# HansiZeng/RIPOR

Measured on AMD Instinct MI355X. Metric: queries/sec, t5-base beam=10 len=32 over 8.8M-doc trie (constrained beam search), higher is better.
Workload: dtype f32 via f16x2-split MFMA (fp32 accumulate)

## Files before the change

### ripor_amd/csrc/gemm_h2.hip

```cpp
#include <algorithm>
#include <cstdio>
#include <type_traits>
#include <hip/hip_fp16.h>

#include <cstdlib>

#include "common.h"
#include "gemm_route.h"

#include <algorithm>
#include <vector>

namespace rpr {

typedef _Float16 f16x8 __attribute__((ext_vector_type(8)));
typedef __bf16 bf16x8 __attribute__((ext_vector_type(8)));
typedef float f32x16 __attribute__((ext_vector_type(16)));
typedef float f32x4 __attribute__((ext_vector_type(4)));
typedef float f32x2 __attribute__((ext_vector_type(2)));
typedef _Float16 f16x2 __attribute__((ext_vector_type(2)));

template <bool M16, int TM, int TN> struct H2Acc { typedef f32x16 type[TM][TN]; };
template <int TM, int TN> struct H2Acc<true, TM, TN> { typedef f32x4 type[2 * TM][2 * TN]; };

// ... 68 lines not shown
      __half* dst = smem + (size_t)buf * ROWS * HBK + 16 * (wave + NW * j) * HBK;
      __builtin_amdgcn_global_load_lds((const __attribute__((address_space(1))) void*)(src[j] + k0),
                                       (__attribute__((address_space(3))) void*)dst, 16, 0, 0);
    }
  };

  f32x16 acc[TM][TN];
#pragma unroll
  for (int i = 0; i < TM; ++i)
#pragma unroll
    for (int j = 0; j < TN; ++j)
#pragma unroll
      for (int r = 0; r < 16; ++r) acc[i][j][r] = 0.f;

  const int frow = lane & 31, sw = (lane >> 2) & 3, hf = lane >> 5;
  const int a_row = wm * (BM / WM) + frow, w_row = 2 * BM + wn * (BN / WN) + frow;

  auto compute = [&](int buf) {
    const __half* base = smem + (size_t)buf * ROWS * HBK;
#pragma unroll
    for (int c = 0; c < HBK / 16; ++c) {
      const int so = ((2 * c + hf) ^ sw) * 8;
      if (BF16) {
        bf16x8 a0[TM], a1[TM], b0[TN], b1[TN];
#pragma unroll
        for (int i = 0; i < TM; ++i) {
          a0[i] = *reinterpret_cast<const bf16x8*>(base + (a_row + i * 32) * HBK + so);
          a1[i] = *reinterpret_cast<const bf16x8*>(base + (BM + a_row + i * 32) * HBK + so);
        }
#pragma unroll
        for (int j = 0; j < TN; ++j) {
          b0[j] = *reinterpret_cast<const bf16x8*>(base + (w_row + j * 32) * HBK + so);
          b1[j] = *reinterpret_cast<const bf16x8*>(base + (BN + w_row + j * 32) * HBK + so);
        }
#pragma unroll
        for (int i = 0; i < TM; ++i)
#pragma unroll
          for (int j = 0; j < TN; ++j) acc[i][j] = __builtin_amdgcn_mfma_f32_32x32x16_bf16(a0[i], b0[j], acc[i][j], 0, 0, 0);
#pragma unroll
        for (int i = 0; i < TM; ++i)
#pragma unroll
          for (int j = 0; j < TN; ++j) acc[i][j] = __builtin_amdgcn_mfma_f32_32x32x16_bf16(a1[i], b1[j], acc[i][j], 0, 0, 0);
        continue;
      }
      f16x8 ah[TM], al[TM], bh[TN], bl[TN];
#pragma unroll
      for (int i = 0; i < TM; ++i) {
        ah[i] = *reinterpret_cast<const f16x8*>(base + (a_row + i * 32) * HBK + so);
        al[i] = *reinterpret_cast<const f16x8*>(base + (BM + a_row + i * 32) * HBK + so);
      }
#pragma unroll
      for (int j = 0; j < TN; ++j) {
        bh[j] = *reinterpret_cast<const f16x8*>(base + (w_row + j * 32) * HBK + so);
        bl[j] = *reinterpret_cast<const f16x8*>(base + (BN + w_row + j * 32) * HBK + so);
      }
#pragma unroll
      for (int i = 0; i < TM; ++i)
#pragma unroll
        for (int j = 0; j < TN; ++j) acc[i][j] = __builtin_amdgcn_mfma_f32_32x32x16_f16(al[i], bh[j], acc[i][j], 0, 0, 0);
#pragma unroll
      for (int i = 0; i < TM; ++i)
#pragma unroll
        for (int j = 0; j < TN; ++j) acc[i][j] = __builtin_amdgcn_mfma_f32_32x32x16_f16(ah[i], bl[j], acc[i][j], 0, 0, 0);
#pragma unroll
      for (int i = 0; i < TM; ++i)
#pragma unroll
        for (int j = 0; j < TN; ++j) acc[i][j] = __builtin_amdgcn_mfma_f32_32x32x16_f16(ah[i], bh[j], acc[i][j], 0, 0, 0);
    }
  };

  if (STAGES == 2) {
    stage(0, 0);
    __syncthreads();
    for (int kt = 0; kt + 1 < nkt; ++kt) {
      stage((kt + 1) & 1, (kt + 1) * KSTEP);
      compute(kt & 1);
      __syncthreads();
    }
    compute((nkt - 1) & 1);
  } else {
    constexpr int AHEAD = STAGES - 1;
    static_assert(PER_WAVE * (AHEAD - 1) <= 63, "vmcnt is a 6-bit counter");
    constexpr int KEEP = PER_WAVE * (AHEAD - 1);
    constexpr int WAIT_KEEP = (KEEP & 15) | ((KEEP >> 4) << 14) | 0x0f70;
    constexpr int WAIT_NONE = 0x0f70;
#pragma unroll
    for (int t = 0; t < AHEAD; ++t)
      if (t < nkt) stage(t, t * KSTEP);
    for (int kt = 0; kt < nkt; ++kt) {
      if (kt + AHEAD - 1 < nkt) __builtin_amdgcn_s_waitcnt(WAIT_KEEP); else __builtin_amdgcn_s_waitcnt(WAIT_NONE);
      __builtin_amdgcn_s_barrier();
      __builtin_amdgcn_sched_barrier(0);
      if (kt + AHEAD < nkt) stage((kt + AHEAD) % STAGES, (kt + AHEAD) * KSTEP);
      compute(kt % STAGES);
      __builtin_amdgcn_sched_barrier(0);
    }
  }

  if (BF16) {
    constexpr int SH = BM / WM, SW = BN / WN;
    static_assert((size_t)BM * BN * sizeof(float) <= sizeof(smem), "the strips of all waves fit the operand buffers");
    __syncthreads();
    float* stg = reinterpret_cast<float*>(smem) + (size_t)wave * (SH * SW);
    const int ncol_ = lane & 31, rsub_ = 4 * (lane >> 5);
#pragma unroll
    for (int i = 0; i < TM; ++i)
#pragma unroll
      for (int j = 0; j < TN; ++j)
#pragma unroll
        for (int r = 0; r < 16; ++r) stg[(i * 32 + (r & 3) + 8 * (r >> 2) + rsub_) * SW + j * 32 + ncol_] = acc[i][j][r];
    __builtin_amdgcn_s_waitcnt(0xc07f);
    __builtin_amdgcn_wave_barrier();
    constexpr int LPR = SW / 4, RPI = 64 / LPR, NK = SH / RPI;
    const int rrow = lane / LPR, rc4 = (lane % LPR) * 4;
    const int mrow0 = bm + wm * SH, n0 = bn + wn * SW + rc4;
    const bool ncol_ok = FULL || n0 < g.N;
    float* outp = g.out[0] + (size_t)blockIdx.y * g.part_stride;
    const int ldo = g.ldo[0];
    const float relu_lo = g.relu ? 0.f : -INFINITY;
    float4 res[NK];
    if (g.resid) {
#pragma unroll
      for (int k = 0; k < NK; ++k) {
        const int m = min(mrow0 + k * RPI + rrow, g.M - 1), nc = ncol_ok ? n0 : 0;
        res[k] = *reinterpret_cast<const float4*>(g.resid + (size_t)m * g.ldr + nc);
      }
    }
#pragma unroll
    for (int k = 0; k < NK; ++k) {
      const int rl = k * RPI + rrow, m = mrow0 + rl;
      float4 v = *reinterpret_cast<const float4*>(stg + rl * SW + rc4);
      v.x = fmaxf(v.x * acc_scale, relu_lo); v.y = fmaxf(v.y * acc_scale, relu_lo);
      v.z = fmaxf(v.z * acc_scale, relu_lo); v.w = fmaxf(v.w * acc_scale, relu_lo);
      if (g.resid) { v.x = res[k].x + v.x; v.y = res[k].y + v.y; v.z = res[k].z + v.z; v.w = res[k].w + v.w; }
      if (ncol_ok && (FULL || m < g.M)) *reinterpret_cast<float4*>(outp + (size_t)m * ldo + n0) = v;
    }
    return;
  }
  int lane_e = lane;
  asm volatile("" : "+v"(lane_e));
  h2_epilogue_256<FULL, TM, TN, WM, WN, BM, BN>(g, acc, smem, wave, lane_e, bm, bn, wm, wn, g.row_ssq ? rs_tile : nullptr, acc_scale);
}

template <bool FULL, int TM, int TN, int WM, int WN, int strip, int BM = 256, int BN = 256, bool BOUT = false, bool M16 = false>
__device__ __forceinline__ void h2_epilogue_strip(const GemmH2Args& g, typename H2Acc<M16, TM, TN>::type& acc, float* stg, int lane, int bm, int bn,
                                                  int wm, int wn, const float* rs_tile, float acc_scale, int Mlim) {
  constexpr int SH = 64, SW = TN * 32;
  const int ncol = lane & 31, rsub = 4 * (lane >> 5);
  if constexpr (M16) {
    const int c16 = lane & 15, r16 = 4 * (lane >> 4);
#pragma unroll
    for (int ii = 0; ii < SH / 16; ++ii)
#pragma unroll
      for (int j = 0; j < 2 * TN; ++j)
#pragma unroll
        for (int r = 0; r < 4; ++r)
          stg[(ii * 16 + r16 + r) * SW + j * 16 + c16] = acc[strip * (SH / 16) + ii][j][r];
  } else
#pragma unroll
    for (int ii = 0; ii < SH / 32; ++ii)
#pragma unroll
      for (int j = 0; j < TN; ++j)
#pragma unroll
        for (int r = 0; r < 16; ++r)
          stg[(ii * 32 + (r & 3) + 8 * (r >> 2) + rsub) * SW + j * 32 + ncol] = acc[strip * (SH / 32) + ii][j][r];
    __builtin_amdgcn_s_waitcnt(0xc07f);
    __builtin_amdgcn_wave_barrier();
    const int mrow0 = bm + wm * (BM / WM) + strip * SH;
    auto planes_path = [&](auto res_tag) __attribute__((always_inline)) {
      constexpr bool RES = decltype(res_tag)::value;
      constexpr int LPR = SW / 8, RPI = 64 / LPR, NK = SH / RPI, KB = RES ? 2 : 4;
      const int rrow = lane / LPR, rc8 = (lane % LPR) * 8;
      const int n0 = bn + wn * (BN / WN) + rc8;
      const bool ncol_ok = FULL || (n0 < g.N);
      const float ps = g.plane_scale;
      float amax = 0.f;
      uint4 rh[RES ? NK : 1], rl_[RES ? NK : 1];
      if (RES) {
#pragma unroll
        for (int k = 0; k < NK; ++k) {
          const int m = min(mrow0 + k * RPI + rrow, Mlim - 1), nc = ncol_ok ? n0 : 0;
          rh[k] = *reinterpret_cast<const uint4*>(g.resid_h + (size_t)m * g.ldrh + nc);
          rl_[k] = *reinterpret_cast<const uint4*>(g.resid_h + g.r_ps + (size_t)m * g.ldrh + nc);
        }
      }
#pragma unroll
      for (int kb = 0; kb < NK; kb += KB) {
        float4 sa[KB], sb[KB];
        float scs[KB];
#pragma unroll
        for (int k = 0; k < KB; ++k) {
          const int rl = (kb + k) * RPI + rrow;
          sa[k] = *reinterpret_cast<const float4*>(stg + rl * SW + rc8);
          sb[k] = *reinterpret_cast<const float4*>(stg + rl * SW + rc8 + 4);
          scs[k] = rs_tile ? rs_tile[wm * (BM / WM) + strip * SH + rl] : 1.0f;
        }
        __builtin_amdgcn_sched_barrier(0);
#pragma unroll
        for (int k = 0; k < KB; ++k) {
          const int rl = (kb + k) * RPI + rrow, m = mrow0 + rl;
          const bool ok = ncol_ok && (FULL || m < Mlim);
          const float sc = rs_tile ? acc_scale * scs[k] : acc_scale;
          f32x2 v[4];
          *reinterpret_cast<float4*>(&v[0]) = sa[k];
          *reinterpret_cast<float4*>(&v[2]) = sb[k];
          f16x2 h[4], l[4];
          f32x2 ss2 = {0.f, 0.f};
          float am = 0.f;
#pragma unroll
          for (int e = 0; e < 4; ++e) {
            f32x2 x = v[e] * sc;
            if (g.relu) { x.x = fmaxf(x.x, 0.f); x.y = fmaxf(x.y, 0.f); }
            if (RES) {
              x += (__builtin_convertvector(reinterpret_cast<const f16x2*>(&rh[RES ? kb + k : 0])[e], f32x2) +
                    __builtin_convertvector(reinterpret_cast<const f16x2*>(&rl_[RES ? kb + k : 0])[e], f32x2)) * (1.0f / X_PLANE_SCALE);
            }
            ss2 += x * x;
            f32x2 xs = x * ps;
            am = fmaxf(am, fmaxf(fabsf(xs.x), fabsf(xs.y)));
            xs.x = __builtin_amdgcn_fmed3f(xs.x, -65504.f, 65504.f);
            xs.y = __builtin_amdgcn_fmed3f(xs.y, -65504.f, 65504.f);
            h[e] = __builtin_convertvector(xs, f16x2);
            l[e] = __builtin_convertvector(xs - __builtin_convertvector(h[e], f32x2), f16x2);
          }
          float ss = ss2.x + ss2.y;
          if (ok) {
            *reinterpret_cast<uint4*>(g.out_h + (size_t)m * g.ldoh + n0) = *reinterpret_cast<uint4*>(h);
            *reinterpret_cast<uint4*>(g.out_h + g.o_ps + (size_t)m * g.ldoh + n0) = *reinterpret_cast<uint4*>(l);
            amax = fmaxf(amax, am);
          }
          if (g.ssq_out) {
            if (!ok) ss = 0.f;
#pragma unroll
            for (int o = LPR / 2; o > 0; o >>= 1) ss += __shfl_xor(ss, o, 64);
            if ((lane % LPR) == 0 && (FULL || m < Mlim)) atomicAdd(g.ssq_out + m, ssq_to_fix(ss, g.sat));
          }
        }
      }
      if (amax > 65504.f && g.sat) *g.sat = 1u;
    };
    auto fp32_path = [&](auto res_tag, auto kv_tag) __attribute__((always_inline)) {
      constexpr bool RES = decltype(res_tag)::value, KVMAP = decltype(kv_tag)::value;
      const float relu_lo = g.relu ? 0.f : -INFINITY;
      constexpr int LPR = SW / 4, RPI = 64 / LPR, NK = SH / RPI, KB = RES ? 4 : 8;
      const int rrow = lane / LPR, rc4 = (lane % LPR) * 4;
      const int n0 = bn + wn * (BN / WN) + rc4;
      const bool ncol_ok = FULL || (n0 < g.N);
      const int oi = ncol_ok ? n0 / g.split_n : 0, on = n0 - oi * g.split_n;
      float* outp = (oi == 0 ? g.out[0] : oi == 1 ? g.out[1] : g.out[2]) + (size_t)blockIdx.y * g.part_stride;
      const int ldo = oi == 0 ? g.ldo[0] : oi == 1 ? g.ldo[1] : g.ldo[2];
      float4 res[RES ? NK : 1];
      if (RES) {
#pragma unroll
        for (int k = 0; k < NK; ++k) {
          const int m = min(mrow0 + k * RPI + rrow, Mlim - 1), nc = ncol_ok ? n0 : 0;
          res[k] = *reinterpret_cast<const float4*>(g.resid + (size_t)m * g.ldr + nc);
        }
      }
#pragma unroll
      for (int kb = 0; kb < NK; kb += KB) {
        float4 st[KB];
        float scs[KB];
#pragma unroll
        for (int k = 0; k < KB; ++k) {
          const int rl = (kb + k) * RPI + rrow;
          st[k] = *reinterpret_cast<const float4*>(stg + rl * SW + rc4);
          scs[k] = rs_tile ? rs_tile[wm * (BM / WM) + strip * SH + rl] : 1.0f;
        }
        __builtin_amdgcn_sched_barrier(0);
#pragma unroll
        for (int k = 0; k < KB; ++k) {
          const int rl = (kb + k) * RPI + rrow, m = mrow0 + rl;
          float4 v = st[k];
          const float sc = acc_scale * scs[k];
          v.x = fmaxf(v.x * sc, relu_lo); v.y = fmaxf(v.y * sc, relu_lo); v.z = fmaxf(v.z * sc, relu_lo); v.w = fmaxf(v.w * sc, relu_lo);
          if (RES) { const float4 r = res[RES ? kb + k : 0]; v.x = r.x + v.x; v.y = r.y + v.y; v.z = r.z + v.z; v.w = r.w + v.w; }
          if (ncol_ok && (FULL || m < Mlim)) {
            const size_t off = KVMAP ? out_off(g, oi, m, ldo, on) : (size_t)m * ldo + on;
            *reinterpret_cast<float4*>(outp + off) = v;
          }
        }
      }
    };
    auto bf16_path = [&](auto mask_tag) __attribute__((always_inline)) {
      constexpr bool MASK = decltype(mask_tag)::value;
      constexpr int LPR = SW / 8, RPI = 64 / LPR, NK = SH / RPI, KB = MASK ? 2 : 4;
      const int rrow = lane / LPR, rc8 = (lane % LPR) * 8;
      const int n0 = bn + wn * (BN / WN) + rc8;
      const float relu_lo = g.relu ? 0.f : -INFINITY;
      __bf16* ob = reinterpret_cast<__bf16*>(g.out_b);
      float* of = g.out[0];
      float4 ma[MASK ? NK : 1], mb[MASK ? NK : 1];
      if (MASK) {
#pragma unroll
        for (int k = 0; k < NK; ++k) {
          const float* mp = g.mask_src + (size_t)(mrow0 + k * RPI + rrow) * g.ldmask + n0;
          ma[k] = *reinterpret_cast<const float4*>(mp);
          mb[k] = *reinterpret_cast<const float4*>(mp + 4);
        }
      }
#pragma unroll
      for (int kb = 0; kb < NK; kb += KB) {
        float4 sa[KB], sb[KB];
#pragma unroll
        for (int k = 0; k < KB; ++k) {
          const int rl = (kb + k) * RPI + rrow;
          sa[k] = *reinterpret_cast<const float4*>(stg + rl * SW + rc8);
          sb[k] = *reinterpret_cast<const float4*>(stg + rl * SW + rc8 + 4);
        }
        __builtin_amdgcn_sched_barrier(0);
#pragma unroll
        for (int k = 0; k < KB; ++k) {
          const int rl = (kb + k) * RPI + rrow, m = mrow0 + rl;
          float v[8] = {sa[k].x, sa[k].y, sa[k].z, sa[k].w, sb[k].x, sb[k].y, sb[k].z, sb[k].w};
#pragma unroll
          for (int e = 0; e < 8; ++e) v[e] = fmaxf(v[e] * acc_scale, relu_lo);
          if (MASK) {
            const float mk[8] = {ma[MASK ? kb + k : 0].x, ma[MASK ? kb + k : 0].y, ma[MASK ? kb + k : 0].z, ma[MASK ? kb + k : 0].w,
                                 mb[MASK ? kb + k : 0].x, mb[MASK ? kb + k : 0].y, mb[MASK ? kb + k : 0].z, mb[MASK ? kb + k : 0].w};
#pragma unroll
            for (int e = 0; e < 8; ++e) v[e] = mk[e] > 0.f ? v[e] : 0.f;
          }
          if (g.out_bt) {
            *reinterpret_cast<float4*>(stg + rl * SW + rc8) = make_float4(v[0], v[1], v[2], v[3]);
            *reinterpret_cast<float4*>(stg + rl * SW + rc8 + 4) = make_float4(v[4], v[5], v[6], v[7]);
          }
          if (ob) {
            __bf16 b[8];
#pragma unroll
            for (int e = 0; e < 8; ++e) b[e] = (__bf16)v[e];
            *reinterpret_cast<uint4*>(ob + (size_t)m * g.ldob + n0) = *reinterpret_cast<uint4*>(b);
          }
          if (of) {
            *reinterpret_cast<float4*>(of + (size_t)m * g.ldo[0] + n0) = make_float4(v[0], v[1], v[2], v[3]);
            *reinterpret_cast<float4*>(of + (size_t)m * g.ldo[0] + n0 + 4) = make_float4(v[4], v[5], v[6], v[7]);
          }
        }
      }
      if (g.out_bt) {
        __builtin_amdgcn_s_waitcnt(0xc07f);
        __builtin_amdgcn_wave_barrier();
        __bf16* obt = reinterpret_cast<__bf16*>(g.out_bt);
        const int c = lane & 31, hrow = 32 * (lane >> 5);
#pragma unroll
        for (int cc = 0; cc < SW; cc += 32) {
          float col[32];
#pragma unroll
          for (int r = 0; r < 32; ++r) col[r] = stg[(hrow + r) * SW + cc + c];
          __bf16 b[32];
#pragma unroll
          for (int r = 0; r < 32; ++r) b[r] = (__bf16)col[r];
          __bf16* dst = obt + (size_t)(bn + wn * (BN / WN) + cc + c) * g.ldobt + mrow0 + hrow;
#pragma unroll
          for (int j = 0; j < 4; ++j) reinterpret_cast<uint4*>(dst)[j] = reinterpret_cast<const uint4*>(b)[j];
        }
      }
    };
    if (BOUT && (g.out_b || g.out_bt)) {
      if (g.mask_src) bf16_path(std::true_type{}); else bf16_path(std::false_type{});
    } else if (g.out_h) {
      if (g.resid_h) planes_path(std::true_type{}); else planes_path(std::false_type{});
    } else {
      if (g.rm_B) { if (g.resid) fp32_path(std::true_type{}, std::true_type{}); else fp32_path(std::false_type{}, std::true_type{}); }
      else if (g.resid) fp32_path(std::true_type{}, std::false_type{});
      else fp32_path(std::false_type{}, std::false_type{});
    }
    __builtin_amdgcn_wave_barrier();
}

template <bool FULL, int TM, int TN, int WM, int WN, int BM, int BN, bool BOUT, bool M16>
__device__ __forceinline__ void h2_epilogue_256(const GemmH2Args& g, typename H2Acc<M16, TM, TN>::type& acc, __half* smem, int wave,
                                                int lane, int bm, int bn, int wm, int wn, const float* rs_tile,
                                                float acc_scale) {
  constexpr int SH = 64;
  __syncthreads();
  const int Mlim = g.m_dev ? min(*g.m_dev - g.m_base, g.M) : g.M;
  constexpr int SW = TN * 32;
  constexpr int NS = TM * 32 / SH;
  float* stg = reinterpret_cast<float*>(smem) + wave * (SH * SW);
  const int ncol = lane & 31, rsub = 4 * (lane >> 5);
  static_assert(NS == 1 || NS == 2, "one or two strips of 64 rows per wave");
  (void)ncol; (void)rsub;
  h2_epilogue_strip<FULL, TM, TN, WM, WN, 0, BM, BN, BOUT, M16>(g, acc, stg, lane, bm, bn, wm, wn, rs_tile, acc_scale, Mlim);
  if (NS == 2) h2_epilogue_strip<FULL, TM, TN, WM, WN, NS - 1, BM, BN, BOUT, M16>(g, acc, stg, lane, bm, bn, wm, wn, rs_tile, acc_scale, Mlim);
}

template <bool FULL, bool BF16 = false, bool M16 = false>
__global__ __launch_bounds__(512, 2) void gemm_h2_pp_kernel(GemmH2Args g, int tiles_m, int tiles_n) {
  static_assert(!(BF16 && M16), "the 16x16x32 body is the split-precision kernel's");
#include "gemm_h2_pp_body.inc"
}

template <bool FULL>
__global__ __launch_bounds__(512, 2) void gemm_h2_pp_group_kernel(const GemmH2Args* __restrict__ table, const int* __restrict__ assign) {
  constexpr bool BF16 = true, M16 = false;
  const int asg = assign[blockIdx.x];
  if (asg < 0) return;
  const GemmH2Args& g = table[asg >> 16];
  const int tiles_m = (g.M + 255) >> 8, tiles_n = (g.N + 255) >> 8;
#define PP_GROUP_TILE (asg & 0xffff)
#include "gemm_h2_pp_body.inc"
#undef PP_GROUP_TILE
}

struct GroupAssign { int n; int v[GemmGroupArgs::MAX_BLOCKS]; };
__global__ void gemm_group_table_kernel(GemmGroupArgs p, GroupAssign a, GemmH2Args* __restrict__ table, int* __restrict__ assign) {
  const int i = threadIdx.x;
  for (int k = i; k < a.n; k += blockDim.x) assign[k] = a.v[k];
  if (i >= p.n) return;
  GemmH2Args g{};
  g.A = p.A[i]; g.W = p.W[i]; g.lda = p.lda; g.ldw = p.ldw;
  g.out[0] = g.out[1] = g.out[2] = p.out[i];
  g.ldo[0] = g.ldo[1] = g.ldo[2] = p.ldo[i];
  g.M = p.M[i]; g.N = p.N[i]; g.K = p.K; g.split_n = p.N[i];
  g.acc_scale = 1.0f; g.plane_scale = 1.0f; g.bf16 = 1;
  table[i] = g;
}

__device__ __forceinline__ int live_rows(const GemmH2Args& g) {
  if (!g.m_dev) return g.M;
  const int md = *g.m_dev;
  if (g.live_hi > 0 && (md <= g.live_lo || md > g.live_hi)) return -1;
  return min(md, g.M);
}

struct EpiIn { unsigned long long ssq; float rf; unsigned int rh, rl; };

__device__ __forceinline__ EpiIn epi_load(const GemmH2Args g, int m, int n, bool mok, bool nok) {
  EpiIn e;
  e.ssq = (g.row_ssq && mok) ? g.row_ssq[m] : 0ull;
  e.rf = (g.resid && mok && nok) ? g.resid[(size_t)m * g.ldr + n] : 0.f;
  e.rh = (g.resid_h && mok && nok) ? (unsigned int)reinterpret_cast<const unsigned short*>(g.resid_h)[(size_t)m * g.ldrh + n] : 0u;
  e.rl = (g.resid_h && mok && nok) ? (unsigned int)reinterpret_cast<const unsigned short*>(g.resid_h)[g.r_ps + (size_t)m * g.ldrh + n] : 0u;
  return e;
}

template <int R, typename RowOf>
__device__ __forceinline__ void epi_fetch(const GemmH2Args g, unsigned long long (&ssq)[R], float (&rf)[R], unsigned int (&rh)[R],
                                          unsigned int (&rl)[R], int n, bool nok, int Mlive, RowOf row) {
#pragma unroll
  for (int r = 0; r < R; ++r) {
    const EpiIn x = epi_load(g, row(r), n, row(r) < Mlive, nok);
    ssq[r] = x.ssq; rf[r] = x.rf; rh[r] = x.rh; rl[r] = x.rl;
  }
}

__device__ __forceinline__ float epi_apply(const GemmH2Args& g, float acc, float acc_scale, const EpiIn& e, int m, int n, bool mok,
                                           bool ok, float* outp, int ldo, int oi, int on) {
  float v = acc * acc_scale;
  if (g.row_ssq && mok) v *= ssq_rsqrt(e.ssq, g.inv_d_fix, g.eps);
  if (g.relu) v = fmaxf(v, 0.f);
  if (g.resid && ok) v = e.rf + v;
  if (g.resid_h && ok) v = x_from_planes(__ushort_as_half((unsigned short)e.rh), __ushort_as_half((unsigned short)e.rl)) + v;
  if (ok) {
    if (g.out_h) {
      __half hi, lo;
      split_f16(v * g.plane_scale, hi, lo, g.sat);
      g.out_h[(size_t)m * g.ldoh + n] = hi;
      g.out_h[g.o_ps + (size_t)m * g.ldoh + n] = lo;
      v = (__half2float(hi) + __half2float(lo)) / g.plane_scale;
    } else {
      outp[out_off(g, oi, m, ldo, on)] = v;
    }
  }
  return v;
}

template <bool FULL>
__global__ __launch_bounds__(256, 1) void gemm_h2_skinny16_kernel(GemmH2Args g, int tiles_n) {
  const float acc_scale = g.dyn_a ? 1.0f / (dyn_plane_scale(*g.dyn_a) * dyn_plane_scale(*g.dyn_b)) : g.acc_scale;
  constexpr int BT = 16, ST = 6, ROWS = 4 * BT, PIECES = ROWS / 16;
  __shared__ __attribute__((aligned(16))) __half smem[4 * ST * ROWS * HBK];
  const int bn = blockIdx.x * BT, bm = blockIdx.y * BT;
  const int Mlive = live_rows(g);
  if (bm >= Mlive) return;
  const int tid = threadIdx.x, lane = tid & 63;
  const int wave = __builtin_amdgcn_readfirstlane(tid >> 6);
  __half* wsm = smem + (size_t)wave * ST * ROWS * HBK;
  const int n = bn + (lane & 15), rsub = 4 * (lane >> 4);
  const bool nok = FULL || n < g.N;
  const auto row = [&](int r) { return bm + rsub + r; };
  unsigned long long e_ssq[4];
  float e_rf[4];
  unsigned int e_rh[4], e_rl[4];
  if (wave == 0) epi_fetch(g, e_ssq, e_rf, e_rh, e_rl, n, nok, Mlive, row);
  const __half* src[PIECES];
#pragma unroll
  for (int j = 0; j < PIECES; ++j) {
    const int lrow = 16 * j + (lane >> 2);
    const int seg = (lane & 3) ^ ((lrow >> 2) & 3);
    const bool is_a = j < 2, second = (j & 1) != 0;
    const __half* base = is_a ? g.A : g.W;
    const size_t plane = second ? (is_a ? g.a_ps : g.w_ps) : 0;
    const int limit = is_a ? g.M : g.N;
    const size_t ld = is_a ? (size_t)g.lda : (size_t)g.ldw;
    int trow = (is_a ? bm : bn) + (lane >> 2);
    if (trow >= limit) trow = limit - 1;
    src[j] = base + plane + (size_t)trow * ld + seg * 8;
  }
  auto stage = [&](int buf, int k0) {
#pragma unroll
    for (int j = 0; j < PIECES; ++j)
      __builtin_amdgcn_global_load_lds((const __attribute__((address_space(1))) void*)(src[j] + k0),
                                       (__attribute__((address_space(3))) void*)(wsm + (size_t)buf * ROWS * HBK + 16 * j * HBK),
                                       16, 0, 0);
  };
  typedef float f32x4 __attribute__((ext_vector_type(4)));
  f32x4 acc = {0.f, 0.f, 0.f, 0.f};
  const int frow = lane & 15, kg = lane >> 4;
  const int so = (kg ^ ((frow >> 2) & 3)) * 8;
  auto compute = [&](int buf) {
    const __half* base = wsm + (size_t)buf * ROWS * HBK + frow * HBK + so;
    const f16x8 ah = *reinterpret_cast<const f16x8*>(base);
    const f16x8 al = *reinterpret_cast<const f16x8*>(base + BT * HBK);
    const f16x8 bh = *reinterpret_cast<const f16x8*>(base + 2 * BT * HBK);
    const f16x8 bl = *reinterpret_cast<const f16x8*>(base + 3 * BT * HBK);
    acc = __builtin_amdgcn_mfma_f32_16x16x32_f16(al, bh, acc, 0, 0, 0);
    acc = __builtin_amdgcn_mfma_f32_16x16x32_f16(ah, bl, acc, 0, 0, 0);
    acc = __builtin_amdgcn_mfma_f32_16x16x32_f16(ah, bh, acc, 0, 0, 0);
  };
  const int nkt = g.K / HBK;
  const int mine = wave < nkt ? (nkt - wave + 3) / 4 : 0;
  constexpr int KEEP = PIECES * (ST - 2);
  constexpr int WAIT_KEEP = (KEEP & 15) | ((KEEP >> 4) << 14) | 0x0f70, WAIT_NONE = 0x0f70;
#pragma unroll
  for (int t = 0; t < ST - 1; ++t)
    if (t < mine) stage(t, (wave + 4 * t) * HBK);
  for (int i = 0; i < mine; ++i) {
    if (i + ST - 2 < mine) __builtin_amdgcn_s_waitcnt(WAIT_KEEP); else __builtin_amdgcn_s_waitcnt(WAIT_NONE);
// ... 461 lines not shown
```

### ripor_amd/csrc/gemm_h2_pp_body.inc

```
  const float acc_scale = g.dyn_a ? 1.0f / (dyn_plane_scale(*g.dyn_a) * dyn_plane_scale(*g.dyn_b)) : g.acc_scale;
  constexpr int BM = 256, BN = 256, WM = 2, WN = 4, NW = 8, TM = 4, TN = 2;
  constexpr int ROWS = 2 * (BM + BN), PER_WAVE = ROWS / 16 / NW;
  __shared__ __attribute__((aligned(16))) __half smem[2 * ROWS * HBK];
  __shared__ float rs_tile[BM];

  int nt = tiles_m * tiles_n;
  if (g.m_dev) {
    if (g.live_hi > 0 && (*g.m_dev <= g.live_lo || *g.m_dev > g.live_hi)) return;
    nt = ((min(*g.m_dev, g.M) + BM - 1) / BM) * tiles_n;
  }
  const int tid = threadIdx.x, lane = tid & 63;
  const int wave = __builtin_amdgcn_readfirstlane(tid >> 6);
  const int wm = wave / WN, wn = wave % WN;
#ifdef PP_GROUP_TILE
  const int xk = 0, xstep = 1, chunk0 = (PP_GROUP_TILE), chunk_n = 1;
#else
  const int xq = nt >> 3, xr = nt & 7, xcd = blockIdx.x & 7, xk = blockIdx.x >> 3, xstep = ((int)gridDim.x - xcd + 7) >> 3;
  const int chunk0 = xcd < xr ? xcd * (xq + 1) : xr * (xq + 1) + (xcd - xr) * xq, chunk_n = xcd < xr ? xq + 1 : xq;
#endif
  int round = 0;
  for (int ti = xk; ti < chunk_n; ti += xstep, ++round) {
  const int bid = chunk0 + ti;
  int tm = bid / tiles_n, tn = bid - tm * tiles_n;
  if (g.tile_cw > 0) {
    const int band_sz = g.tile_rb * tiles_n, band = bid / band_sz, rem = bid - band * band_sz;
    const int rb = min(g.tile_rb, nt / tiles_n - band * g.tile_rb);
    const int gsz = rb * g.tile_cw, gi = rem / gsz, r2 = rem - gi * gsz;
    const int c0 = gi * g.tile_cw, cwg = min(g.tile_cw, tiles_n - c0);
    const int pr = r2 / cwg;
    tm = band * g.tile_rb + pr; tn = c0 + (r2 - pr * cwg);
  }
  const int bm = tm * BM, bn = tn * BN;
  if (g.row_ssq && tid < BM) {
    const int m = bm + tid;
    rs_tile[tid] = (m < g.M) ? ssq_rsqrt(g.row_ssq[m], g.inv_d_fix, g.eps) : 1.f;
  }

  constexpr int KSTEP = BF16 ? 2 * HBK : HBK;
  int nkt = g.K / KSTEP, kbeg = 0;
  if (g.ksplit > 1) {
    const int per = (nkt + g.ksplit - 1) / g.ksplit;
    kbeg = blockIdx.y * per;
    nkt = min(per, nkt - kbeg);
  }
  int lane_t = lane;
  asm volatile("" : "+v"(lane_t));
  const __half* src[PER_WAVE];
#define PP_SRC_SETUP(dst, lane_x, bm_x, bn_x)                                                                         \
  _Pragma("unroll") for (int j = 0; j < PER_WAVE; ++j) {                                                              \
    const int grow = 16 * (wave + NW * j);                             \
    const int lrow = grow + ((lane_x) >> 2);                                                                          \
    const int seg = ((lane_x) & 3) ^ ((lrow >> 2) & 3);                                                               \
    const bool is_a = grow < 2 * BM, second = is_a ? grow >= BM : grow >= 2 * BM + BN;                                \
    const __half* base = is_a ? g.A : g.W;                                                                            \
    const size_t plane = second ? (BF16 ? (size_t)HBK : (is_a ? g.a_ps : g.w_ps)) : 0;                                \
    const int limit = is_a ? g.M : g.N;                                                                               \
    const size_t ld = is_a ? (size_t)g.lda : (size_t)g.ldw;                                                           \
    int trow = (is_a ? (bm_x) + lrow - (second ? BM : 0) : (bn_x) + lrow - 2 * BM - (second ? BN : 0));               \
    if (!FULL && trow >= limit) trow = limit - 1;                                                                     \
    dst[j] = base + plane + (size_t)trow * ld + seg * 8 + (size_t)kbeg * KSTEP;                                       \
  }
  PP_SRC_SETUP(src, lane_t, bm, bn)
#define PP_PIECE(buf, k0, j)                                                                                   \
  __builtin_amdgcn_global_load_lds((const __attribute__((address_space(1))) void*)(src[j] + (k0)),             \
                                   (__attribute__((address_space(3))) void*)(smem + (size_t)(buf) * ROWS * HBK + \
                                                                             16 * (wave + NW * (j)) * HBK),     \
                                   16, 0, 0)

  f32x16 acc[TM][TN];
#pragma unroll
  for (int i = 0; i < TM; ++i)
#pragma unroll
    for (int j = 0; j < TN; ++j)
#pragma unroll
      for (int r = 0; r < 16; ++r) acc[i][j][r] = 0.f;

  const int frow = lane & 31, sw = (lane >> 2) & 3, hf = lane >> 5;
  const int a_row = wm * (BM / WM) + frow, w_row = 2 * BM + wn * (BN / WN) + frow;
  const int so0 = ((0 + hf) ^ sw) * 8, so1 = ((2 + hf) ^ sw) * 8;

  f16x8 ah0, ah1, al0, al1, bh0, bh1, bl0, bl1;
  f16x8 ah2, ah3, al2, al3;
  f32x4 acc16[8][4];
  f16x8 wh2, wh3, wl2, wl3;
  const int a_row16 = wm * (BM / WM) + (lane & 15), w_row16 = 2 * BM + wn * (BN / WN) + (lane & 15);
  const int so16 = ((lane >> 4) ^ ((lane >> 2) & 3)) * 8;
  if constexpr (M16) {
#pragma unroll
    for (int i = 0; i < 8; ++i)
#pragma unroll
      for (int j = 0; j < 4; ++j) acc16[i][j] = f32x4{0.f, 0.f, 0.f, 0.f};
  }
#define PP_LOAD_W(buf, so)                                                                              \
  {                                                                                                     \
    const __half* base_ = smem + (size_t)(buf) * ROWS * HBK;                                            \
    bh0 = *reinterpret_cast<const f16x8*>(base_ + (w_row) * HBK + (so));                                \
    bh1 = *reinterpret_cast<const f16x8*>(base_ + (w_row + 32) * HBK + (so));                           \
    bl0 = *reinterpret_cast<const f16x8*>(base_ + (BN + w_row) * HBK + (so));                           \
    bl1 = *reinterpret_cast<const f16x8*>(base_ + (BN + w_row + 32) * HBK + (so));                      \
  }
#define PP_LOAD_A(buf, so, i0)                                                                          \
  {                                                                                                     \
    const __half* base_ = smem + (size_t)(buf) * ROWS * HBK;                                            \
    ah0 = *reinterpret_cast<const f16x8*>(base_ + (a_row + (i0) * 32) * HBK + (so));                    \
    ah1 = *reinterpret_cast<const f16x8*>(base_ + (a_row + (i0) * 32 + 32) * HBK + (so));               \
    al0 = *reinterpret_cast<const f16x8*>(base_ + (BM + a_row + (i0) * 32) * HBK + (so));               \
    al1 = *reinterpret_cast<const f16x8*>(base_ + (BM + a_row + (i0) * 32 + 32) * HBK + (so));          \
  }
#define PP_LOAD_A4(buf, so)                                                                             \
  {                                                                                                     \
    const __half* base_ = smem + (size_t)(buf) * ROWS * HBK;                                            \
    ah0 = *reinterpret_cast<const f16x8*>(base_ + (a_row) * HBK + (so));                                \
    ah1 = *reinterpret_cast<const f16x8*>(base_ + (a_row + 32) * HBK + (so));                           \
    ah2 = *reinterpret_cast<const f16x8*>(base_ + (a_row + 64) * HBK + (so));                           \
    ah3 = *reinterpret_cast<const f16x8*>(base_ + (a_row + 96) * HBK + (so));                           \
    al0 = *reinterpret_cast<const f16x8*>(base_ + (BM + a_row) * HBK + (so));                           \
    al1 = *reinterpret_cast<const f16x8*>(base_ + (BM + a_row + 32) * HBK + (so));                      \
    al2 = *reinterpret_cast<const f16x8*>(base_ + (BM + a_row + 64) * HBK + (so));                      \
    al3 = *reinterpret_cast<const f16x8*>(base_ + (BM + a_row + 96) * HBK + (so));                      \
  }
#define PP_MFMA(a, b, c)                                                                                 \
  do {                                                                                                   \
    if (BF16) c = __builtin_amdgcn_mfma_f32_32x32x16_bf16(__builtin_bit_cast(bf16x8, a), __builtin_bit_cast(bf16x8, b), c, 0, 0, 0); \
    else c = __builtin_amdgcn_mfma_f32_32x32x16_f16(a, b, c, 0, 0, 0);                                   \
  } while (0)
#define PP_MMA(i0, D1, D2, D3)                                                                          \
  {                                                                                                     \
    if (BF16) {                              \
      PP_MFMA(al0, bl0, acc[(i0)][0]); PP_MFMA(al0, bl1, acc[(i0)][1]);                                 \
      __builtin_amdgcn_sched_barrier(0); D1; __builtin_amdgcn_sched_barrier(0);                         \
      PP_MFMA(al1, bl0, acc[(i0) + 1][0]); PP_MFMA(al1, bl1, acc[(i0) + 1][1]);                         \
      __builtin_amdgcn_sched_barrier(0); D2; __builtin_amdgcn_sched_barrier(0);                         \
      PP_MFMA(ah0, bh0, acc[(i0)][0]); PP_MFMA(ah0, bh1, acc[(i0)][1]);                                 \
      __builtin_amdgcn_sched_barrier(0); D3; __builtin_amdgcn_sched_barrier(0);                         \
      PP_MFMA(ah1, bh0, acc[(i0) + 1][0]); PP_MFMA(ah1, bh1, acc[(i0) + 1][1]);                         \
    } else {                                                                                            \
    PP_MFMA(al0, bh0, acc[(i0)][0]); PP_MFMA(al0, bh1, acc[(i0)][1]);                                   \
    __builtin_amdgcn_sched_barrier(0); D1; __builtin_amdgcn_sched_barrier(0);                           \
    PP_MFMA(al1, bh0, acc[(i0) + 1][0]); PP_MFMA(al1, bh1, acc[(i0) + 1][1]);                           \
    PP_MFMA(ah0, bl0, acc[(i0)][0]); PP_MFMA(ah0, bl1, acc[(i0)][1]);                                   \
    __builtin_amdgcn_sched_barrier(0); D2; __builtin_amdgcn_sched_barrier(0);                           \
    PP_MFMA(ah1, bl0, acc[(i0) + 1][0]); PP_MFMA(ah1, bl1, acc[(i0) + 1][1]);                           \
    PP_MFMA(ah0, bh0, acc[(i0)][0]); PP_MFMA(ah0, bh1, acc[(i0)][1]);                                   \
    __builtin_amdgcn_sched_barrier(0); D3; __builtin_amdgcn_sched_barrier(0);                           \
    PP_MFMA(ah1, bh0, acc[(i0) + 1][0]); PP_MFMA(ah1, bh1, acc[(i0) + 1][1]);                           \
    }                                                                                                   \
  }
#define PP_SB __builtin_amdgcn_sched_barrier(0)
#define PP_MMA8(A0, A1, A2, A3, B0, B1, Da, Db, Dc)                                                     \
    PP_MFMA(A0, B0, acc[0][0]); PP_MFMA(A0, B1, acc[0][1]); PP_MFMA(A1, B0, acc[1][0]);                 \
    PP_SB; Da; PP_SB;                                                                                   \
    PP_MFMA(A1, B1, acc[1][1]); PP_MFMA(A2, B0, acc[2][0]); PP_MFMA(A2, B1, acc[2][1]);                 \
    PP_SB; Db; PP_SB;                                                                                   \
    PP_MFMA(A3, B0, acc[3][0]); PP_MFMA(A3, B1, acc[3][1]);                                             \
    PP_SB; Dc; PP_SB;
#define PP_MMA24(D0, D1, D2, D3, D4, D5, D6, D7)                                                        \
  {                                                                                                     \
    if (BF16) {                              \
      PP_MMA8(al0, al1, al2, al3, bl0, bl1, D0, D1, D2)                                                 \
      PP_SB; D3; D4; PP_SB;                                                                             \
      PP_MMA8(ah0, ah1, ah2, ah3, bh0, bh1, D5, D6, D7)                                                 \
    } else {                                                                                            \
      PP_MMA8(al0, al1, al2, al3, bh0, bh1, D0, D1, D2)                                                 \
      PP_MMA8(ah0, ah1, ah2, ah3, bl0, bl1, D3, D4, D5)                                                 \
      PP_MMA8(ah0, ah1, ah2, ah3, bh0, bh1, D6, D7, (void)0)                                            \
    }                                                                                                   \
  }
#define PP_DMA(j) if (more) PP_PIECE(nxt, k1, j)
#define PP_DMA_M(j) PP_DMA(j)
#define PP_L_END(waitimm, ph)                                                                           \
  __builtin_amdgcn_sched_barrier(0);                                                                    \
  __builtin_amdgcn_s_waitcnt(waitimm);                                                                  \
  __builtin_amdgcn_s_barrier();                                                                         \
  __builtin_amdgcn_sched_barrier(0);                                                                    \
  __builtin_amdgcn_s_setprio(1)
#define PP_M_END(ph)                                                                                    \
  __builtin_amdgcn_sched_barrier(0);                                                                    \
  __builtin_amdgcn_s_setprio(0);                                                                        \
  __builtin_amdgcn_s_barrier();                                                                         \
  __builtin_amdgcn_sched_barrier(0)
  constexpr int WAIT_LGKM = 0xc07f, WAIT_ALL = 0x0070;
  constexpr int WAIT_VM4 = 0x0074;
#define PP16_LOAD_W(buf)                                                                                \
  {                                                                                                     \
    const __half* base_ = smem + (size_t)(buf) * ROWS * HBK + so16;                                     \
    bh0 = *reinterpret_cast<const f16x8*>(base_ + (w_row16) * HBK);                                     \
    bh1 = *reinterpret_cast<const f16x8*>(base_ + (w_row16 + 16) * HBK);                                \
    wh2 = *reinterpret_cast<const f16x8*>(base_ + (w_row16 + 32) * HBK);                                \
    wh3 = *reinterpret_cast<const f16x8*>(base_ + (w_row16 + 48) * HBK);                                \
    bl0 = *reinterpret_cast<const f16x8*>(base_ + (BN + w_row16) * HBK);                                \
    bl1 = *reinterpret_cast<const f16x8*>(base_ + (BN + w_row16 + 16) * HBK);                           \
    wl2 = *reinterpret_cast<const f16x8*>(base_ + (BN + w_row16 + 32) * HBK);                           \
    wl3 = *reinterpret_cast<const f16x8*>(base_ + (BN + w_row16 + 48) * HBK);                           \
  }
#define PP16_LOAD_A(buf, ph)                                                                            \
  {                                                                                                     \
    const __half* base_ = smem + (size_t)(buf) * ROWS * HBK + so16;                                     \
    ah0 = *reinterpret_cast<const f16x8*>(base_ + (a_row16 + (ph) * 64) * HBK);                         \
    ah1 = *reinterpret_cast<const f16x8*>(base_ + (a_row16 + (ph) * 64 + 16) * HBK);                    \
    ah2 = *reinterpret_cast<const f16x8*>(base_ + (a_row16 + (ph) * 64 + 32) * HBK);                    \
    ah3 = *reinterpret_cast<const f16x8*>(base_ + (a_row16 + (ph) * 64 + 48) * HBK);                    \
    al0 = *reinterpret_cast<const f16x8*>(base_ + (BM + a_row16 + (ph) * 64) * HBK);                    \
    al1 = *reinterpret_cast<const f16x8*>(base_ + (BM + a_row16 + (ph) * 64 + 16) * HBK);               \
    al2 = *reinterpret_cast<const f16x8*>(base_ + (BM + a_row16 + (ph) * 64 + 32) * HBK);               \
    al3 = *reinterpret_cast<const f16x8*>(base_ + (BM + a_row16 + (ph) * 64 + 48) * HBK);               \
  }
#define PP16_MFMA(a, b, c) c = __builtin_amdgcn_mfma_f32_16x16x32_f16(a, b, c, 0, 0, 0)
#define PP16_ROW(A, i, B0, B1, B2, B3)                                                                  \
    PP16_MFMA(A, B0, acc16[i][0]); PP16_MFMA(A, B1, acc16[i][1]); PP16_MFMA(A, B2, acc16[i][2]); PP16_MFMA(A, B3, acc16[i][3]);
#define PP16_MMA16(i0, A0, A1, A2, A3, B0, B1, B2, B3, Da, Db, Dc)                                      \
    PP16_ROW(A0, (i0), B0, B1, B2, B3)                                                                  \
    PP16_MFMA(A1, B0, acc16[(i0) + 1][0]); PP16_MFMA(A1, B1, acc16[(i0) + 1][1]);                       \
    PP_SB; Da; PP_SB;                                                                                   \
    PP16_MFMA(A1, B2, acc16[(i0) + 1][2]); PP16_MFMA(A1, B3, acc16[(i0) + 1][3]);                       \
    PP16_ROW(A2, (i0) + 2, B0, B1, B2, B3)                                                              \
    PP_SB; Db; PP_SB;                                                                                   \
    PP16_ROW(A3, (i0) + 3, B0, B1, B2, B3)                                                              \
    PP_SB; Dc; PP_SB;
#define PP16_MMA48(i0, D0, D1, D2, D3, D4, D5, D6, D7)                                                  \
  {                                                                                                     \
    PP16_MMA16(i0, al0, al1, al2, al3, bh0, bh1, wh2, wh3, D0, D1, D2)                                  \
    PP16_MMA16(i0, ah0, ah1, ah2, ah3, bl0, bl1, wl2, wl3, D3, D4, D5)                                  \
    PP16_MMA16(i0, ah0, ah1, ah2, ah3, bh0, bh1, wh2, wh3, D6, D7, (void)0)                             \
  }

#pragma unroll
  for (int j = 0; j < PER_WAVE; ++j) PP_PIECE(0, 0, j);
  if (BF16 && nkt > 1) {
    PP_PIECE(1, KSTEP, 0); PP_PIECE(1, KSTEP, 1); PP_PIECE(1, KSTEP, 4); PP_PIECE(1, KSTEP, 5);
    __builtin_amdgcn_s_waitcnt(WAIT_VM4);
  } else {
    __builtin_amdgcn_s_waitcnt(WAIT_ALL);
  }
  __builtin_amdgcn_s_barrier();
  __builtin_amdgcn_sched_barrier(0);
  if (wm == 1) __builtin_amdgcn_s_barrier();
  __builtin_amdgcn_sched_barrier(0);
  if (BF16) {
    for (int kt = 0; kt < nkt; ++kt) {
// ... 102 lines not shown
```

Before: 5258.

## Permute W rows in M16 GEMM so epilogue writes directly from registers

After: 5323 (median of 6 runs). +1.2%, better.

```diff
diff --git a/ripor_amd/csrc/gemm_h2.hip b/ripor_amd/csrc/gemm_h2.hip
--- a/ripor_amd/csrc/gemm_h2.hip
+++ b/ripor_amd/csrc/gemm_h2.hip
@@ -244,10 +244,9 @@
 #pragma unroll
     for (int ii = 0; ii < SH / 16; ++ii)
 #pragma unroll
-      for (int j = 0; j < 2 * TN; ++j)
-#pragma unroll
-        for (int r = 0; r < 4; ++r)
-          stg[(ii * 16 + r16 + r) * SW + j * 16 + c16] = acc[strip * (SH / 16) + ii][j][r];
+      for (int r = 0; r < 4; ++r)
+        *reinterpret_cast<f32x4*>(stg + (ii * 16 + r16 + r) * SW + 4 * c16) =
+            f32x4{acc[strip * (SH / 16) + ii][0][r], acc[strip * (SH / 16) + ii][1][r], acc[strip * (SH / 16) + ii][2][r], acc[strip * (SH / 16) + ii][3][r]};
   } else
 #pragma unroll
     for (int ii = 0; ii < SH / 32; ++ii)
@@ -450,7 +449,7 @@
     };
     if (BOUT && (g.out_b || g.out_bt)) {
       if (g.mask_src) bf16_path(std::true_type{}); else bf16_path(std::false_type{});
-    } else if (g.out_h) {
+    } else if (!M16 && g.out_h) {
       if (g.resid_h) planes_path(std::true_type{}); else planes_path(std::false_type{});
     } else {
       if (g.rm_B) { if (g.resid) fp32_path(std::true_type{}, std::true_type{}); else fp32_path(std::false_type{}, std::true_type{}); }
@@ -458,6 +457,133 @@
       else fp32_path(std::false_type{}, std::false_type{});
     }
     __builtin_amdgcn_wave_barrier();
+}
+
+template <int CTRL>
+__device__ __forceinline__ float h2_dpp(float x) {
+  return __builtin_bit_cast(float, __builtin_amdgcn_update_dpp(0, __builtin_bit_cast(int, x), CTRL, 0xf, 0xf, false));
+}
+constexpr int DPP_ROR8 = 0x128, DPP_XOR1 = 0xB1, DPP_XOR2 = 0x4E, DPP_XOR3 = 0x1B, DPP_HALF_MIRROR = 0x141;
+
+template <bool FULL, bool RES>
+__device__ __forceinline__ void h2_direct16_planes(const GemmH2Args& g, f32x4 (&acc)[8][4], int lane, int bm, int bn, int wm, int wn,
+                                                   const float* rs_tile, float acc_scale, int Mlim) {
+  const int c = lane & 15, gq = lane >> 4;
+  const bool hi = c >= 8;
+  const int lrow0 = wm * 128 + 4 * gq + (hi ? 1 : 0), mrow0 = bm + lrow0;
+  const int n0 = bn + wn * 64 + 8 * (c & 7);
+  const bool ncol_ok = FULL || (n0 < g.N);
+  const float ps = g.plane_scale;
+  float amax = 0.f;
+  float scs[16];
+  auto load = [&](auto it_c, uint4 (&q)[4]) __attribute__((always_inline)) {
+    constexpr int it = decltype(it_c)::value;
+#pragma unroll
+    for (int p = 0; p < 2; ++p) {
+      scs[2 * it + p] = rs_tile ? rs_tile[lrow0 + 16 * it + 2 * p] : 1.0f;
+      if (RES) {
+        const int m = min(mrow0 + 16 * it + 2 * p, Mlim - 1), nc = ncol_ok ? n0 : 0;
+        q[2 * p] = *reinterpret_cast<const uint4*>(g.resid_h + (size_t)m * g.ldrh + nc);
+        q[2 * p + 1] = *reinterpret_cast<const uint4*>(g.resid_h + g.r_ps + (size_t)m * g.ldrh + nc);
+      }
+    }
+  };
+  auto tile = [&](auto it_c, const uint4 (&q)[4]) __attribute__((always_inline)) {
+    constexpr int it = decltype(it_c)::value;
+#pragma unroll
+    for (int p = 0; p < 2; ++p) {
+      f32x4 v0, v1;
+#pragma unroll
+      for (int j = 0; j < 4; ++j) {
+        const float got = h2_dpp<DPP_ROR8>(hi ? acc[it][j][2 * p] : acc[it][j][2 * p + 1]);
+        v0[j] = hi ? got : acc[it][j][2 * p];
+        v1[j] = hi ? acc[it][j][2 * p + 1] : got;
+      }
+      const int m = mrow0 + 16 * it + 2 * p;
+      const bool ok = ncol_ok && (FULL || m < Mlim);
+      const float sc = rs_tile ? acc_scale * scs[2 * it + p] : acc_scale;
+      f32x2 v[4] = {{v0[0], v0[1]}, {v0[2], v0[3]}, {v1[0], v1[1]}, {v1[2], v1[3]}};
+      f16x2 h[4], l[4];
+      f32x2 ss2 = {0.f, 0.f};
+      float am = 0.f;
+#pragma unroll
+      for (int e = 0; e < 4; ++e) {
+        f32x2 x = v[e] * sc;
+        if (g.relu) { x.x = fmaxf(x.x, 0.f); x.y = fmaxf(x.y, 0.f); }
+        if (RES) {
+          x += (__builtin_convertvector(reinterpret_cast<const f16x2*>(&q[2 * p])[e], f32x2) +
+                __builtin_convertvector(reinterpret_cast<const f16x2*>(&q[2 * p + 1])[e], f32x2)) * (1.0f / X_PLANE_SCALE);
+        }
+        ss2 += x * x;
+        f32x2 xs = x * ps;
+        am = fmaxf(am, fmaxf(fabsf(xs.x), fabsf(xs.y)));
+        xs.x = __builtin_amdgcn_fmed3f(xs.x, -65504.f, 65504.f);
+        xs.y = __builtin_amdgcn_fmed3f(xs.y, -65504.f, 65504.f);
+        h[e] = __builtin_convertvector(xs, f16x2);
+        l[e] = __builtin_convertvector(xs - __builtin_convertvector(h[e], f32x2), f16x2);
+      }
+      float ss = ss2.x + ss2.y;
+      if (ok) {
+        *reinterpret_cast<uint4*>(g.out_h + (size_t)m * g.ldoh + n0) = *reinterpret_cast<uint4*>(h);
+        *reinterpret_cast<uint4*>(g.out_h + g.o_ps + (size_t)m * g.ldoh + n0) = *reinterpret_cast<uint4*>(l);
+        amax = fmaxf(amax, am);
+      }
+      if (g.ssq_out) {
+        if (!ok) ss = 0.f;
+        ss += h2_dpp<DPP_XOR3>(h2_dpp<DPP_HALF_MIRROR>(ss));
+        ss += h2_dpp<DPP_XOR2>(ss);
+        ss += h2_dpp<DPP_XOR1>(ss);
+        if ((c & 7) == 0 && (FULL || m < Mlim)) atomicAdd(g.ssq_out + m, ssq_to_fix(ss, g.sat));
+      }
+    }
+  };
+#define H2_PIN_AMAX() asm volatile("" : "+v"(amax)); __builtin_amdgcn_sched_barrier(0)
+  using std::integral_constant;
+  uint4 qa[4], qb[4], qc[4];
+#define H2_T(it, q) tile(integral_constant<int, it>{}, q); H2_PIN_AMAX()
+#define H2_L(it, q) load(integral_constant<int, it>{}, q); __builtin_amdgcn_sched_barrier(0)
+  H2_L(0, qa); H2_L(1, qb); H2_L(2, qc);
+  H2_T(0, qa); H2_L(3, qa);
+  H2_T(1, qb); H2_L(4, qb);
+  H2_T(2, qc); H2_L(5, qc);
+  H2_T(3, qa); H2_L(6, qa);
+  H2_T(4, qb); H2_L(7, qb);
+  H2_T(5, qc); H2_T(6, qa); H2_T(7, qb);
+#undef H2_T
+#undef H2_L
+#undef H2_PIN_AMAX
+  if (amax > 65504.f && g.sat) *g.sat = 1u;
+}
+
+template <bool FULL>
+__device__ __forceinline__ void h2_direct16_fp32(const GemmH2Args& g, f32x4 (&acc)[8][4], int lane, int bm, int bn, int wm, int wn,
+                                                 const float* rs_tile, float acc_scale, int Mlim) {
+  const int c = lane & 15, gq = lane >> 4;
+  const int lrow0 = wm * 128 + 4 * gq, mrow0 = bm + lrow0;
+  const float relu_lo = g.relu ? 0.f : -INFINITY;
+  const int n0 = bn + wn * 64 + 4 * c;
+  const bool ncol_ok = FULL || (n0 < g.N);
+  const int oi = ncol_ok ? n0 / g.split_n : 0, on = n0 - oi * g.split_n;
+  float* outp = (oi == 0 ? g.out[0] : oi == 1 ? g.out[1] : g.out[2]) + (size_t)blockIdx.y * g.part_stride;
+  const int ldo = oi == 0 ? g.ldo[0] : oi == 1 ? g.ldo[1] : g.ldo[2];
+#pragma unroll
+  for (int ib = 0; ib < 8; ib += 4) {
+    f32x4 scs[4];
+#pragma unroll
+    for (int k = 0; k < 4; ++k)
+      scs[k] = rs_tile ? *reinterpret_cast<const f32x4*>(rs_tile + lrow0 + 16 * (ib + k)) : f32x4{1.f, 1.f, 1.f, 1.f};
+    __builtin_amdgcn_sched_barrier(0);
+#pragma unroll
+    for (int k = 0; k < 4; ++k)
+#pragma unroll
+      for (int r = 0; r < 4; ++r) {
+        const int m = mrow0 + 16 * (ib + k) + r;
+        const float sc = acc_scale * scs[k][r];
+        f32x4 v = {acc[ib + k][0][r], acc[ib + k][1][r], acc[ib + k][2][r], acc[ib + k][3][r]};
+        v[0] = fmaxf(v[0] * sc, relu_lo); v[1] = fmaxf(v[1] * sc, relu_lo); v[2] = fmaxf(v[2] * sc, relu_lo); v[3] = fmaxf(v[3] * sc, relu_lo);
+        if (ncol_ok && (FULL || m < Mlim)) *reinterpret_cast<f32x4*>(outp + (size_t)m * ldo + on) = v;
+      }
+  }
 }
 
 template <bool FULL, int TM, int TN, int WM, int WN, int BM, int BN, bool BOUT, bool M16>
@@ -467,6 +593,17 @@
   constexpr int SH = 64;
   __syncthreads();
   const int Mlim = g.m_dev ? min(*g.m_dev - g.m_base, g.M) : g.M;
+  if constexpr (M16) {
+    if (g.out_h) {
+      if (g.resid_h) h2_direct16_planes<FULL, true>(g, acc, lane, bm, bn, wm, wn, rs_tile, acc_scale, Mlim);
+      else h2_direct16_planes<FULL, false>(g, acc, lane, bm, bn, wm, wn, rs_tile, acc_scale, Mlim);
+      return;
+    }
+    if (!g.rm_B && !g.resid) {
+      h2_direct16_fp32<FULL>(g, acc, lane, bm, bn, wm, wn, rs_tile, acc_scale, Mlim);
+      return;
+    }
+  }
   constexpr int SW = TN * 32;
   constexpr int NS = TM * 32 / SH;
   float* stg = reinterpret_cast<float*>(smem) + wave * (SH * SW);
diff --git a/ripor_amd/csrc/gemm_h2_pp_body.inc b/ripor_amd/csrc/gemm_h2_pp_body.inc
--- a/ripor_amd/csrc/gemm_h2_pp_body.inc
+++ b/ripor_amd/csrc/gemm_h2_pp_body.inc
@@ -57,6 +57,10 @@
     const int limit = is_a ? g.M : g.N;                                                                               \
     const size_t ld = is_a ? (size_t)g.lda : (size_t)g.ldw;                                                           \
     int trow = (is_a ? (bm_x) + lrow - (second ? BM : 0) : (bn_x) + lrow - 2 * BM - (second ? BN : 0));               \
+    if (M16 && !is_a) {    \
+      const int wrow = trow - (bn_x), wc = wrow & 15, wj = (wrow >> 4) & 3;                                           \
+      trow = (bn_x) + ((wrow & ~63) | (g.out_h ? 8 * (wc & 7) + 4 * (wc >> 3) + wj : 4 * wc + wj));                   \
+    }                                                                                                                 \
     if (!FULL && trow >= limit) trow = limit - 1;                                                                     \
     dst[j] = base + plane + (size_t)trow * ld + seg * 8 + (size_t)kbeg * KSTEP;                                       \
   }
@@ -83,8 +87,8 @@
   f16x8 ah2, ah3, al2, al3;
   f32x4 acc16[8][4];
   f16x8 wh2, wh3, wl2, wl3;
-  const int a_row16 = wm * (BM / WM) + (lane & 15), w_row16 = 2 * BM + wn * (BN / WN) + (lane & 15);
-  const int so16 = ((lane >> 4) ^ ((lane >> 2) & 3)) * 8;
+  const int a_row16 = wm * (BM / WM) + (lane_t & 15), w_row16 = 2 * BM + wn * (BN / WN) + (lane_t & 15);
+  const int so16 = ((lane_t >> 4) ^ ((lane_t >> 2) & 3)) * 8;
   if constexpr (M16) {
 #pragma unroll
     for (int i = 0; i < 8; ++i)
```
